# METHODS-Group/ProximalGalerkin

Hardware: AMD Instinct MI355X
Metric: proximal-Newton iterations/sec, 2048^2 P1 obstacle (LVPP Newton inner loop) (higher is better)
Workload: dtype f64; 1 GPU; 2048x2048 right-diagonal P1 obstacle problem on [-1,1]^2, phi_set obstacle, f=0, settings B: alpha double_exponential, alpha_max 100, tol 0.0001; snes_rtol 1e-6, Newton linear solves to true relative residual 1e-10; mixed_unknowns=8396802, step=one full LVPP solve from the zero state, parallelism=single

## Files before the change

proximalgalerkin_amd/csrc/pgx_api.hip:

```cpp
#include <algorithm>
#include <atomic>
#include <chrono>
#include <thread>
#include <cmath>
#include <cstdio>
#include <cstring>
#include <deque>
#include <map>
#include <mutex>
#include <string>
#include <vector>

#include "../../include/pgx.h"
#include "../../include/pgx_nd.h"
#include "pgx_comm.h"
#include "pgx_internal.h"

static thread_local std::string g_create_error;

struct DistLevel {
  int g, glo, H, ghi;
};
struct Dist {
  bool on = false;
  pgx_comm* comm = nullptr;
  int rank = 0, size = 1, ldist = 0, global_ny = 0;
  std::vector<DistLevel> L;
  GridLevel view{};
  int view_row0 = 0, view_glo = 0, view_H = 0, view_own0 = 0;
  long long n_halo = 0, n_allreduce = 0, n_vcycle = 0, n_krylov = 0;
  double* view_S = nullptr;
  size_t own_off = 0, own_cnt = 0;
  size_t eb = 0, eown_off = 0, eown_cnt = 0;
  size_t nk_field() const { return own_cnt + eown_cnt; }
  int cell0 = 0, ncell_own = 0;
  double *sb = nullptr, *wc = nullptr;
};

struct pgx_handle {
  int device = 0;
  Dist dist;
  hipStream_t st = nullptr;
  std::string err;
  int n = 0, nc = 0, nx = 0, ny = 0, nnz = 0;
  int degree = 1;
  int nd = 0;
  bool structured = false;
  QuadTab q{};
  double f = 0.0, alpha = 1.0;
  double* coords = nullptr;
  int32_t* cells = nullptr;
  uint8_t* mask = nullptr;
  double *gbc = nullptr, *bphi = nullptr;
  int32_t *rowptr = nullptr, *colm = nullptr, *v2c_ptr = nullptr, *v2c_ent = nullptr, *v2c_pos = nullptr;
  std::vector<int32_t> h_rowptr, h_col;
  size_t fill_lds = 0;
  double *Kv = nullptr, *Mv = nullptr, *Dv = nullptr;
  bool jac_valid = false;
  double* geoq = nullptr;
  float2* zf_out = nullptr;
  int z_f32 = 1;
  int f32_dbf16 = 1;
  bool dv_lean = false;
  int32_t *s_rowptr = nullptr, *s_colm = nullptr;
  double *s_K = nullptr, *s_M = nullptr, *s_D = nullptr;
  int s_nnz = 0;
  size_t s_fill_lds = 0;
  int32_t* s_blk = nullptr;
  int s_nblk = 0, spmv_bal = 1;
  uint8_t* s_code = nullptr;
  double* s_tab = nullptr;
  int s_ntab = 0, spmv_dict = 1;
  std::vector<int32_t> s_h_rowptr, s_h_col;
  QuadTab2 q2{};
  int32_t *cdofs = nullptr, *p2_v2c_ptr = nullptr, *p2_v2c_ent = nullptr, *p2_v2c_pos = nullptr;
  int32_t *v2e_ptr = nullptr, *v2e = nullptr, *edge_ends = nullptr;
  double *p2_xu = nullptr, *p2_xp = nullptr, *p2_ru = nullptr, *p2_rp = nullptr;
  double* p2_stash = nullptr;
  double *c1_bu = nullptr, *c1_bp = nullptr, *c1_xu = nullptr, *c1_xp = nullptr;
  int patch_nn = 0, p2_patch = 1, patch_nu = 2;
  int p2_fallback_its = 60, p2_fallbacks = 0;
  double patch_omega = 0.8;
  bool patch_fresh = false;
  std::vector<int32_t> patch_dof_host;
  int32_t *pdof = nullptr, *ppos = nullptr;
  void* pinv = nullptr;
  int patch_f32 = 1;
  struct P2St {
    int state = 0, enable = 1, dist_enable = 1, select = 1, i0 = 0, ni = 0, j0 = 0, nj = 0, nframe = 0, ref_rows[4] = {0, 0, 0, 0};
    P2StTab tab;
    double K[46];
    double* Dst = nullptr;
    float* Dstf = nullptr;
    int32_t* frame = nullptr;
    bool fresh = false;
  } p2st;
  float* s_Df = nullptr;
  int p2_resid_f32 = 1;
  int patch_sym = 1;
  double *p2_su = nullptr, *p2_sp = nullptr;
  double *x = nullptr, *xk = nullptr, *F = nullptr, *dx = nullptr, *xw = nullptr, *rhs = nullptr;
  int restart = 0;
  double *V = nullptr, *Z = nullptr, *w = nullptr, *d_small = nullptr, *partials = nullptr, *partials2 = nullptr;
  double* h_small = nullptr;
  double* h_small_dev = nullptr;
  unsigned long long* h_seq = nullptr;
  unsigned long long* h_seq_dev = nullptr;
  unsigned long long seq = 0;
  int lean_d = 1;
  int spmv_d4 = 1;
  int lazy_norm = 1;
  double rhs_scale = 1.0;
  const float* rhs_f32 = nullptr;
  int v_f32 = 1;
  double v_f32_gain = 1e-4;
  double v_f32_max = 1e30;
  int v_f32_min = 1000000;
  bool v_f32_off = false;
  int host_poll = 1;
  int gs_wide = 16;
  int fused_publish = 1;
  int fused_resid = 1;
  int lean_rhs = 1;
  int fused_step = 1;
  std::vector<GridLevel> lev;
  double *tmp_u = nullptr, *tmp_p = nullptr, *res_u = nullptr, *res_p = nullptr;
  double omega_now = 0.0;
  int coarse_sweeps = 4;
  int tail_start = -1;
  int xcd_remap = 2;
  int tail_verts = 1100;
  int spmv_stream = 1;
  int nu_coarse = 0;
  int fused_k3 = 1;
  int fused_legs = 1;
  int fused_min = 4000;
  int cgs_selective = 1;
  long cgs_skipped = 0, cgs_total = 0;
  double cgs_eta2 = 1e-4;
  TailArgs tail{};
  pgx_nd* lu = nullptr;
  pgx_comm* lu_comm = nullptr;
  double* Jmix = nullptr;
  bool dh_interior = false;
  int stag_its = 12;
  double stag_gain = 1e-4;
  int smooth_d32 = 0;
  int k6_max = 0;
  int mg_f32 = 1;
  int f32_min = 4000;
  int f32_k6_max = 300000;
  int f32_rr_max = 300000;
  int resid_grid = 1;
  int spmv_stencil = 1;
  bool lu_active = false;
  bool check_replicas = false;
  double *obs_partials = nullptr, *d_out6 = nullptr;
  int obs_blocks = 0;
  bool prof = false;
  double ms[8] = {0, 0, 0, 0, 0, 0, 0, 0};
  hipEvent_t e0 = nullptr, e1 = nullptr;
  std::vector<void*> allocs;
};

#define HIPCHK(call)                                                                            \
  do {                                                                                          \
    hipError_t e_ = (call);                                                                     \
    if (e_ != hipSuccess) {                                                                     \
      h->err = std::string(#call) + ": " + hipGetErrorString(e_);                               \
      return PGX_EHIP;                                                                          \
    }                                                                                           \
  } while (0)

template <typename T>
static int dalloc(pgx_handle* h, T** p, size_t count) {
  void* q = nullptr;
  hipError_t e = hipMalloc(&q, std::max<size_t>(count, 1) * sizeof(T));
  if (e != hipSuccess) {
    h->err = std::string("hipMalloc: ") + hipGetErrorString(e);
    return PGX_ENOMEM;
  }
  h->allocs.push_back(q);
  *p = (T*)q;
  return PGX_OK;
}
#define DALLOC(p, count)                         \
  do {                                           \
    int rc_ = dalloc(h, &(p), (size_t)(count));  \
    if (rc_) return rc_;                         \
  } while (0)

struct PhaseTimer {
  pgx_handle* h;
  int slot;
  PhaseTimer(pgx_handle* h_, int s) : h(h_), slot(s) {
    static const char* const names[8] = {"pgx:residual", "pgx:jacobian", "pgx:mg_setup/lu_factor", "pgx:spmv", "pgx:precond",
                                         "pgx:orthogonalise", "pgx:observables", "pgx:newton_solve"};
    pgx_roctx(names[s & 7]);
    if (h->prof) hipEventRecord(h->e0, h->st);
  }
  ~PhaseTimer() {
    pgx_roctx(nullptr);
    if (h->prof) {
      hipEventRecord(h->e1, h->st);
      hipEventSynchronize(h->e1);
      float ms = 0;
      hipEventElapsedTime(&ms, h->e0, h->e1);
      h->ms[slot] += ms;
    }
  }
};

namespace {
std::mutex g_tune_mu;
std::atomic<int> g_tune_gen{0};
std::map<std::string, const std::string*>& tune_table() {
  static std::map<std::string, const std::string*> t;
  return t;
}
std::deque<std::string>& tune_pool() {
  static std::deque<std::string> p;
  return p;
}
}
const char* pgx_tune(const char* name) {
  std::lock_guard<std::mutex> lk(g_tune_mu);
  auto& t = tune_table();
  auto it = t.find(name);
  return it == t.end() ? nullptr : it->second->c_str();
}
int pgx_tune_gen() { return g_tune_gen.load(std::memory_order_acquire); }
extern "C" int pgx_tuning_set(const char* key, const char* value) {
  if (!key || strncmp(key, "PGX_", 4) != 0) return PGX_EINVAL;
  std::lock_guard<std::mutex> lk(g_tune_mu);
  if (value) {
    const std::string* interned = nullptr;
    for (const std::string& s : tune_pool())
      if (s == value) interned = &s;
    if (!interned) {
      tune_pool().emplace_back(value);
      interned = &tune_pool().back();
    }
    tune_table()[key] = interned;
  } else {
    tune_table().erase(key);
  }
  g_tune_gen.fetch_add(1, std::memory_order_release);
  return PGX_OK;
}

extern "C" void pgx_default_opts(pgx_snes_opts* o) {
  o->snes_rtol = 1e-8;
  o->snes_atol = 1e-50;
  o->snes_stol = 1e-8;
  o->snes_divtol = 1e4;
  o->snes_max_it = 50;
  o->ksp_rtol = 0.0;
  o->ksp_max_it = 200;
  o->ksp_restart = 30;
  o->mg_nu = 6;
  o->mg_omega = 0.75;
  o->monitor = 0;
  o->pc_type = 0;
  o->linesearch = 0;
}

extern "C" const char* pgx_last_error(const pgx_handle* h) { return h ? h->err.c_str() : g_create_error.c_str(); }

static int build_plan(pgx_handle* h, const pgx_mesh* m, const std::vector<uint8_t>& hmask) {
  const int n = m->n_vertices, nc = m->n_cells;
  std::vector<int32_t> vptr(n + 1, 0);
  for (int c = 0; c < nc; ++c)
    for (int a = 0; a < 3; ++a) {
      const int v = m->cells[3 * c + a];
      if (v < 0 || v >= n) {
        h->err = "cell vertex id out of range";
        return PGX_EINVAL;
      }
      vptr[v + 1]++;
    }
  for (int i = 0; i < n; ++i) vptr[i + 1] += vptr[i];
  std::vector<int32_t> vent(vptr[n]), fillp(vptr.begin(), vptr.end() - 1);
  for (int c = 0; c < nc; ++c)
    for (int a = 0; a < 3; ++a) vent[fillp[m->cells[3 * c + a]]++] = c * 4 + a;
  std::vector<int32_t>& rowptr = h->h_rowptr;
  std::vector<int32_t>& col = h->h_col;
  rowptr.assign(n + 1, 0);
  col.clear();
  col.reserve((size_t)n * 7);
  std::vector<int32_t> tmp;
  for (int i = 0; i < n; ++i) {
    tmp.clear();
    for (int k = vptr[i]; k < vptr[i + 1]; ++k) {
      const int c = vent[k] >> 2;
      tmp.push_back(m->cells[3 * c]);
      tmp.push_back(m->cells[3 * c + 1]);
      tmp.push_back(m->cells[3 * c + 2]);
    }
    if (tmp.empty()) tmp.push_back(i);
    std::sort(tmp.begin(), tmp.end());
    tmp.erase(std::unique(tmp.begin(), tmp.end()), tmp.end());
    if (tmp.size() > 255) {
      h->err = "vertex degree > 255 unsupported";
      return PGX_EINVAL;
// ... 1401 lines not shown
    PhaseTimer t(h, 1);
    if (h->degree == 2) {
      pgxk_fill_rows_p2(h->st, 2, h->nd, h->s_fill_lds, h->s_rowptr, h->p2_v2c_ptr, h->p2_v2c_ent, h->p2_v2c_pos,
                        h->cdofs, h->coords, x + h->nd, h->q2, h->s_D, h->geoq);
      pgxk_fill_rows_p1_Dp2(h->st, h->n, h->fill_lds, h->rowptr, h->v2c_ptr, h->v2c_ent, h->v2c_pos, h->cdofs, h->coords,
                            x + h->nd, h->q2, h->Dv, h->geoq);
    } else if (h->resid_grid && h->structured && !h->lev.empty() && h->lev[0].uniform) {
      pgxk_resid_fill_grid(h->st, 1, h->lev[0], h->fill_lds, h->rowptr, h->v2c_ptr, h->v2c_ent, h->v2c_pos, h->cells, h->coords,
                           h->mask, h->gbc, h->bphi, x, h->xk, h->alpha, h->f, h->q, h->w, h->Dv, 1);
      h->dh_interior = true;
      h->dv_lean = false;
      have_d = true;
    } else {
      pgxk_fill_rows(h->st, 2, h->n, h->fill_lds, h->rowptr, h->v2c_ptr, h->v2c_ent, h->v2c_pos, h->cells, h->coords,
                     x + h->n, h->q, h->Dv, h->geoq);
    }
  }
  if (h->structured) {
    PhaseTimer t(h, 2);
    pgxk_csr_to_stencil_h(h->st, h->n, h->nx + 1, h->rowptr, h->colm, h->Dv, h->lev[0].Dh,
                          (have_d && h->degree == 1 && h->dh_interior) ? h->lev[0].ny : 0);
    h->dh_interior = false;
    if (h->lev[0].Dh32) pgxk_to_float(h->st, (size_t)4 * h->n, h->lev[0].Dh, h->lev[0].Dh32);
    if (h->lev[0].f32) pgxk_f_pack_d(h->st, h->lev[0]);
    if (h->lev[0].Dd4) pgxk_pack_d4(h->st, h->lev[0]);
    const int ld = h->dist.on ? h->dist.ldist : 0;
    for (size_t l = 1; l < h->lev.size(); ++l) {
      if (h->dist.on && (int)l == ld) {
        const Dist& D = h->dist;
        const GridLevel& G = h->lev[l];
#ifdef PGX_DSTEN_FLOAT
        h->err = "PGX_DSTEN_FLOAT builds do not support sharded handles";
        return PGX_EINVAL;
#else
        pgxk_rap7h(h->st, h->lev[l - 1], h->lev[l - 1].Dh, D.view, D.view_S);
        pgxk_view_to_global(h->st, 4, D.view.n, G.n, G.nx + 1, D.view_row0, D.view_own0, D.view_H, D.view_S, G.Dh);
        const int rc = allreduce_dev(h, G.Dh, (size_t)4 * G.n);
        if (rc) return rc;
#endif
      } else {
        pgxk_rap7h(h->st, h->lev[l - 1], h->lev[l - 1].Dh, h->lev[l], h->lev[l].Dh);
      }
      if (h->lev[l].f32) pgxk_f_pack_d(h->st, h->lev[l]);
    }
  }
  h->jac_valid = true;
  h->patch_fresh = false;
  h->p2st.fresh = false;
  return PGX_OK;
}

static bool p2st_ready(pgx_handle* h) {
  pgx_handle::P2St& S = h->p2st;
  if (S.state == 0 || !S.select || (h->dist.on && !S.dist_enable) || !h->s_K || !h->s_D) return false;
  static const int nt[4] = {19, 9, 9, 9}, off[4] = {0, 19, 28, 37};
  const size_t G = (size_t)h->n;
  if (S.state == 1) {
    S.state = 0;
    const std::vector<int32_t>& rp = h->s_h_rowptr;
    double kmax = 0.0, mmax = 0.0;
    for (int t = 0; t < 4; ++t) {
      const int p = rp[S.ref_rows[t]];
      if (hipMemcpy(S.K + off[t], h->s_K + p, sizeof(double) * nt[t], hipMemcpyDeviceToHost) != hipSuccess ||
          hipMemcpy(S.tab.M + off[t], h->s_M + p, sizeof(double) * nt[t], hipMemcpyDeviceToHost) != hipSuccess)
        return false;
    }
    for (int e = 0; e < 46; ++e) kmax = std::max(kmax, std::fabs(S.K[e])), mmax = std::max(mmax, std::fabs(S.tab.M[e]));
    S.tab.kmax = kmax, S.tab.mmax = mmax;
    for (int e = 0; e < 46; ++e) S.tab.aK[e] = S.K[e];
    int* d_fail = nullptr;
    if (hipMalloc((void**)&d_fail, sizeof(int)) != hipSuccess) return false;
    hipMemsetAsync(d_fail, 0, sizeof(int), h->st);
    pgxk_p2st_check(h->st, S.tab, h->nx, h->n, S.i0, S.ni, S.j0, S.nj, 1.0, 1e-12, h->s_rowptr, h->s_K, h->s_M, d_fail);
    int fail = 1;
    const hipError_t e1 = hipMemcpyAsync(&fail, d_fail, sizeof(int), hipMemcpyDeviceToHost, h->st);
    const hipError_t e2 = hipStreamSynchronize(h->st);
    hipFree(d_fail);
    if (e1 != hipSuccess || e2 != hipSuccess || fail) return false;
    void* q = nullptr;
    if (hipMalloc(&q, sizeof(double) * 46 * G) != hipSuccess) {
      (void)hipGetLastError();
      return false;
    }
    h->allocs.push_back(q);
    S.Dst = (double*)q;
    if (h->p2_resid_f32) {
      if (hipMalloc(&q, sizeof(float) * 46 * G) == hipSuccess) {
        h->allocs.push_back(q);
        S.Dstf = (float*)q;
      } else {
        (void)hipGetLastError();
      }
    }
    S.state = 2;
  }
  if (!S.fresh) {
    pgxk_p2st_pack(h->st, h->nx, h->n, S.i0, S.ni, S.j0, S.nj, G, h->s_rowptr, h->s_D, S.Dst, 0);
    if (S.Dstf) pgxk_p2st_pack(h->st, h->nx, h->n, S.i0, S.ni, S.j0, S.nj, G, h->s_rowptr, h->s_D, S.Dstf, 1);
    S.fresh = true;
  }
  for (int e = 0; e < 46; ++e) S.tab.aK[e] = h->alpha * S.K[e];
  return true;
}
static void p2st_apply(pgx_handle* h, const double* xu, const double* xp, const double* bu, const double* bp, double* yu, double* yp,
                       bool inner) {
  pgx_handle::P2St& S = h->p2st;
  const bool f32 = inner && S.Dstf;
  pgxk_p2st_apply(h->st, S.tab, h->nx, h->n, S.i0, S.ni, S.j0, S.nj, (size_t)h->n, f32 ? (const void*)S.Dstf : (const void*)S.Dst, f32, xu,
                  xp, bu, bp, yu, yp);
  pgxk_p2_rows_csr(h->st, S.nframe, S.frame, h->s_rowptr, h->s_colm, h->s_K, h->s_M, h->s_D, h->alpha, h->mask, xu, xp, bu, bp, yu, yp);
}

static void level_apply(pgx_handle* h, int l, int mode, const double* xu, const double* xp, const double* bu,
                        const double* bp, double omega, int first, double* yu, double* yp);
static void spmv_dev(pgx_handle* h, const double* x, double* y) {
  if (h->degree == 2 && h->spmv_stream && h->spmv_bal && p2st_ready(h)) {
    static PgxTuneInt bench_inner("PGX_P2ST_BENCH_INNER", 0);
    p2st_apply(h, x, x + h->nd, nullptr, nullptr, y, y + h->nd, bench_inner.get() != 0);
    return;
  }
  if (h->spmv_stencil && h->structured && h->degree == 1) {
    if (h->spmv_stencil == 2)
      level_apply(h, 0, 0, x, x + h->nd, nullptr, nullptr, 0.0, 0, y, y + h->nd);
    else
      pgxk_st_spmv(h->st, h->lev[0], h->alpha, x, x + h->nd, h->xcd_remap ? 1 : 0, y, y + h->nd);
    return;
  }
  if (h->spmv_stream && h->spmv_bal && h->s_blk)
    pgxk_bspmv_bal(h->st, h->nd, h->s_nblk, h->s_blk, h->s_rowptr, h->s_colm, h->s_K, h->s_M, h->s_code, h->s_tab, h->s_D, h->alpha, h->mask, x,
                   x + h->nd, nullptr, nullptr, h->xcd_remap ? 1 : 0, y, y + h->nd);
  else if (h->spmv_stream && 2 * h->s_fill_lds <= 100 * 1024)
    pgxk_bspmv_stream(h->st, h->nd, h->s_fill_lds, h->s_rowptr, h->s_colm, h->s_K, h->s_M, h->s_D, h->alpha, h->mask, x,
                      x + h->nd, h->xcd_remap ? 1 : 0, y, y + h->nd);
  else
    pgxk_bspmv(h->st, 0, h->nd, h->s_rowptr, h->s_colm, h->s_K, h->s_M, h->s_D, h->alpha, x, x + h->nd, nullptr,
               nullptr, 0.0, h->xcd_remap, y, y + h->nd);
}

static void level_apply(pgx_handle* h, int l, int mode, const double* xu, const double* xp, const double* bu,
                        const double* bp, double omega, int first, double* yu, double* yp) {
  if (l == 0 && !h->structured)
    pgxk_bspmv(h->st, mode, h->n, h->rowptr, h->colm, h->Kv, h->Mv, h->Dv, h->alpha, xu, xp, bu, bp, omega,
               first | h->xcd_remap, yu, yp);
  else
    pgxk_st_apply(h->st, mode, h->lev[l], h->alpha, xu, xp, bu, bp, omega, first | h->xcd_remap, yu, yp);
}

static void vcycle(pgx_handle* h, int l, const double* bu, const double* bp, double* outu, double* outp, int nu, double omega);

static const float2* vcycle_f(pgx_handle* h, int l, const double* bu, const double* bp, double* outu, double* outp, int nu,
                              double omega) {
  GridLevel& L = h->lev[l];
  GridLevel& C = h->lev[l + 1];
  const int K = (nu == 6 && L.n <= h->f32_k6_max && L.n <= h->f32_rr_max) ? 6 : ((nu % 3 == 0 && h->fused_k3) ? 3 : 2);
  const int nl = nu / K;
  const int remap = h->xcd_remap ? 1 : 0;
  float2 *cu = L.xf, *ou = L.xf2;
  const bool fuse = L.n <= h->f32_rr_max;
  float2* const cbf = C.f32 ? C.bf : nullptr;
  double* const cb64u = C.f32 ? nullptr : C.bu;
  double* const cb64p = C.f32 ? nullptr : C.bp;
  {
    const bool rr = fuse && nl == 1;
    const double bscale = (l == 0 && bu) ? h->rhs_scale : 1.0;
    const float* const b32 = (l == 0 && bu) ? h->rhs_f32 : nullptr;
    pgxk_f_smooth(h->st, K, 1, L, h->alpha, nullptr, bu, bp, rr ? &C : nullptr, nullptr, nullptr, nullptr, omega, remap, cu, nullptr,
                  nullptr, rr ? cbf : nullptr, rr ? cb64u : nullptr, rr ? cb64p : nullptr, bscale, b32, b32 ? b32 + L.n : nullptr);
  }
  for (int s = 1; s < nl; ++s) {
    const bool rr = fuse && s + 1 == nl;
    pgxk_f_smooth(h->st, K, 0, L, h->alpha, cu, nullptr, nullptr, rr ? &C : nullptr, nullptr, nullptr, nullptr, omega, remap, ou, nullptr,
                  nullptr, rr ? cbf : nullptr, rr ? cb64u : nullptr, rr ? cb64p : nullptr);
    std::swap(cu, ou);
  }
  if (!fuse) pgxk_f_resid_restrict(h->st, L, h->alpha, cu, C, remap, cbf, cb64u, cb64p);
  const float2* cf = nullptr;
  const double *cdu = nullptr, *cdp = nullptr;
  if (C.f32) {
    cf = vcycle_f(h, l + 1, nullptr, nullptr, nullptr, nullptr, nu, omega);
  } else {
    vcycle(h, l + 1, C.bu, C.bp, C.xu, C.xp, nu, omega);
    cdu = C.xu;
    cdp = C.xp;
  }
  for (int s = 0; s < nl; ++s) {
    const bool lastl = s + 1 == nl;
    float2* const zf = (lastl && l == 0) ? h->zf_out : nullptr;
    const bool out64 = lastl && outu && !zf;
    pgxk_f_smooth(h->st, K, 0, L, h->alpha, cu, nullptr, nullptr, s == 0 ? &C : nullptr, s == 0 ? cf : nullptr, s == 0 ? cdu : nullptr,
                  s == 0 ? cdp : nullptr, omega, remap, zf ? zf : ou, out64 ? outu : nullptr, out64 ? outp : nullptr);
    if (zf) return zf;
    std::swap(cu, ou);
  }
  return cu;
}
static inline bool f32_cycle_ok(const pgx_handle* h, int l, int nu) {
  return h->lev[l].f32 && h->fused_legs && l + 1 < (int)h->lev.size() && nu >= 2 && (nu % 2 == 0 || (nu % 3 == 0 && h->fused_k3));
}

static void vcycle(pgx_handle* h, int l, const double* bu, const double* bp, double* outu, double* outp, int nu,
                   double omega) {
  GridLevel& L = h->lev[l];
  if (f32_cycle_ok(h, l, nu)) {
    vcycle_f(h, l, bu, bp, outu, outp, nu, omega);
    return;
  }
  if (l > 0 && l == h->tail_start) {
    h->tail.nu = (h->nu_coarse > 0) ? std::min(nu, h->nu_coarse) : nu;
    h->tail.omega = omega;
    h->tail.alpha = h->alpha;
    h->tail.coarse_sweeps = h->coarse_sweeps;
    pgxk_mg_tail(h->st, h->tail);
    return;
  }
  const bool last = (l + 1 == (int)h->lev.size());
  double* Au = outu;
  double* Ap = outp;
  double* Bu = (l == 0) ? h->tmp_u : L.xu2;
  double* Bp = (l == 0) ? h->tmp_p : L.xp2;
  double* ru = (l == 0) ? h->res_u : L.ru;
  double* rp = (l == 0) ? h->res_p : L.rp;
  const int Kf = (nu % 3 == 0 && h->fused_k3) ? 3 : (nu % 2 == 0 ? 2 : 0);
  if (h->structured && !last && Kf && h->fused_legs && L.n >= h->fused_min) {
    GridLevel& C = h->lev[l + 1];
    const int remap = h->xcd_remap ? 1 : 0;
    const int Kl = (Kf == 3 && nu % 6 == 0 && L.n <= h->k6_max && pgxk_st_smooth6_ok(L)) ? 6 : Kf;
    const int nl = nu / Kl;
    double *cu = Bu, *cp = Bp, *ou = Au, *op = Ap;
    pgxk_st_smoothK(h->st, Kl, 0, L, h->alpha, nullptr, nullptr, nullptr, nullptr, nullptr, bu, bp, omega, remap, cu, cp);
    for (int s = 1; s < nl; ++s) {
      pgxk_st_smoothK(h->st, Kl, 1, L, h->alpha, cu, cp, nullptr, nullptr, nullptr, bu, bp, omega, remap, ou, op);
      std::swap(cu, ou);
      std::swap(cp, op);
    }
    pgxk_st_resid_restrict(h->st, L, h->alpha, cu, cp, bu, bp, C, remap, C.bu, C.bp);
    vcycle(h, l + 1, C.bu, C.bp, C.xu, C.xp, nu, omega);
    pgxk_st_smoothK(h->st, Kl, 1, L, h->alpha, cu, cp, &C, C.xu, C.xp, bu, bp, omega, remap, ou, op);
    std::swap(cu, ou);
    std::swap(cp, op);
    for (int s = 1; s < nl; ++s) {
      pgxk_st_smoothK(h->st, Kl, 1, L, h->alpha, cu, cp, nullptr, nullptr, nullptr, bu, bp, omega, remap, ou, op);
      std::swap(cu, ou);
      std::swap(cp, op);
    }
    if (cu != Au) {
      hipMemcpyAsync(Au, cu, sizeof(double) * L.n, hipMemcpyDeviceToDevice, h->st);
      hipMemcpyAsync(Ap, cp, sizeof(double) * L.n, hipMemcpyDeviceToDevice, h->st);
    }
    return;
  }
  if (l > 0 && h->nu_coarse > 0) nu = std::min(nu, h->nu_coarse);
  const int total = last ? (h->lev.size() == 1 ? 2 * nu : h->coarse_sweeps) : 2 * nu;
  bool toA = (total % 2) == 1;
  const double *cu = nullptr, *cp = nullptr;
  auto sweep = [&](int first) {
    double* tu = toA ? Au : Bu;
    double* tp = toA ? Ap : Bp;
    level_apply(h, l, 2, cu, cp, bu, bp, omega, first, tu, tp);
    cu = tu;
    cp = tp;
    toA = !toA;
  };
  if (last) {
    for (int s = 0; s < total; ++s) sweep(s == 0);
    return;
  }
  for (int s = 0; s < nu; ++s) sweep(s == 0);
  level_apply(h, l, 1, cu, cp, bu, bp, 0.0, 0, ru, rp);
  GridLevel& C = h->lev[l + 1];
  pgxk_restrict(h->st, L, ru, rp, C, C.bu, C.bp);
  vcycle(h, l + 1, C.bu, C.bp, C.xu, C.xp, nu, omega);
  pgxk_prolong_add(h->st, C, C.xu, C.xp, L, (double*)cu, (double*)cp);
  for (int s = 0; s < nu; ++s) sweep(0);
}

static int vcycle_dist_f(pgx_handle* h, int l, double* bu, double* bp, double* outu, double* outp, int need_out, int nu, double omega,
                         const float2** res);
static int vcycle_dist(pgx_handle* h, int l, double* bu, double* bp, double* outu, double* outp, int need_out, int nu,
                       double omega) {
  Dist& D = h->dist;
  GridLevel& L = h->lev[l];
  if (L.f32 && h->fused_legs) return vcycle_dist_f(h, l, bu, bp, outu, outp, need_out, nu, omega, nullptr);
  const int g = D.L[l].g;
  const int K = (nu % 3 == 0 && g >= 3 && h->fused_k3) ? 3 : 2;
  if (nu % K) {
    h->err = "sharded V-cycle: mg_nu must be even (or a multiple of 3 with deep enough ghost rows)";
    return PGX_EINVAL;
  }
  const int remap = h->xcd_remap ? 1 : 0;
  const int nl = nu / K;
  int rc = halo_level(h, l, bu, bp);
  if (rc) return rc;
  double *cu = (l == 0) ? h->tmp_u : L.xu2, *cp = (l == 0) ? h->tmp_p : L.xp2, *ou = outu, *op = outp;
  int xv;
  pgxk_st_smoothK(h->st, K, 0, L, h->alpha, nullptr, nullptr, nullptr, nullptr, nullptr, bu, bp, omega, remap, cu, cp);
  xv = g - K;
  auto more = [&](const GridLevel* C, const double* ccu, const double* ccp) -> int {
    if (xv < K) {
      const int r = halo_level(h, l, cu, cp);
      if (r) return r;
      xv = g;
    }
    pgxk_st_smoothK(h->st, K, 1, L, h->alpha, cu, cp, C, ccu, ccp, bu, bp, omega, remap, ou, op);
    std::swap(cu, ou);
    std::swap(cp, op);
    xv -= K;
    return PGX_OK;
// ... 1213 lines not shown
```

proximalgalerkin_amd/csrc/pgx_mg32.hip:

```cpp
#include <algorithm>

#include "pgx_internal.h"
#include "pgx_stencil.h"

#define F32_BLOCK 512
#ifndef F32_LEAN
#define F32_LEAN 0
#endif
#ifndef F32_WAVES_EU
#define F32_WAVES_EU 2
#endif
#define F32_RR_CYB 2
#define F32_TB 2

__device__ __forceinline__ float lane_shr1f(float x) {
  int v = __float_as_int(x);
  v = __builtin_amdgcn_update_dpp(v, v, 0x138, 0xf, 0xf, false);
  return __int_as_float(v);
}

typedef float f_v2f __attribute__((ext_vector_type(2)));
typedef __bf16 f_v2bf __attribute__((ext_vector_type(2)));
__device__ __forceinline__ uint32_t f_pack_bf16x2(float lo, float hi) {
  const f_v2f f = {lo, hi};
  return __builtin_bit_cast(uint32_t, __builtin_convertvector(f, f_v2bf));
}
__device__ __forceinline__ void f_pack_d(float4 q, float4& out) { out = q; }
__device__ __forceinline__ void f_pack_d(float4 q, uint2& out) { out = make_uint2(f_pack_bf16x2(q.x, q.y), f_pack_bf16x2(q.z, q.w)); }
__device__ __forceinline__ float4 f_unpack_d(float4 q) { return q; }
__device__ __forceinline__ float4 f_unpack_d(uint2 w) {
  return make_float4(__uint_as_float(w.x << 16), __uint_as_float(w.x & 0xffff0000u), __uint_as_float(w.y << 16),
                     __uint_as_float(w.y & 0xffff0000u));
}
__device__ __forceinline__ void f_zero_d(float4& q) { q = make_float4(0.f, 0.f, 0.f, 0.f); }
__device__ __forceinline__ void f_zero_d(uint2& w) { w = make_uint2(0u, 0u); }

template <class DT>
__global__ void __launch_bounds__(256) k_f_pack_d(int n, const dsten_t* __restrict__ Dh, DT* __restrict__ Dq) {
  const int v = blockIdx.x * blockDim.x + threadIdx.x;
  if (v >= n) return;
  const float big = 1e30f;
  f_pack_d(make_float4(fminf((float)Dh[v], big), fminf((float)Dh[(size_t)n + v], big), fminf((float)Dh[2 * (size_t)n + v], big),
                       fminf((float)Dh[3 * (size_t)n + v], big)),
           Dq[v]);
}
void pgxk_f_pack_d(hipStream_t st, const GridLevel& L) {
  if (L.dbf16)
    hipLaunchKernelGGL(k_f_pack_d<uint2>, dim3((L.n + 255) / 256), dim3(256), 0, st, L.n, L.Dh, (uint2*)L.Dq);
  else
    hipLaunchKernelGGL(k_f_pack_d<float4>, dim3((L.n + 255) / 256), dim3(256), 0, st, L.n, L.Dh, (float4*)L.Dq);
}

struct FCoef {
  float kv[7], mv[7], dv[7];
  int rowbc;
};
struct FConst {
  float kc[7], mc[7];
  float k0, k1, k3, k5, m0, m1, m3, m5;
  int uniform;
};
static inline FConst make_fconst(const GridLevel& L, double alpha) {
  FConst c;
  for (int s = 0; s < 7; ++s) {
    c.kc[s] = (float)alpha * (float)L.Kc[s];
    c.mc[s] = (float)L.Mc[s];
  }
  const float a = (float)alpha;
  c.k0 = a * (float)L.Kc[0];
  c.k1 = a * (float)(0.5 * (L.Kc[1] + L.Kc[2]));
  c.k3 = a * (float)(0.5 * (L.Kc[3] + L.Kc[4]));
  c.k5 = a * (float)(0.5 * (L.Kc[5] + L.Kc[6]));
  c.m0 = (float)L.Mc[0];
  c.m1 = (float)(0.5 * (L.Mc[1] + L.Mc[2]));
  c.m3 = (float)(0.5 * (L.Mc[3] + L.Mc[4]));
  c.m5 = (float)(0.5 * (L.Mc[5] + L.Mc[6]));
  c.uniform = L.uniform;
  return c;
}
template <class DT>
__device__ __forceinline__ void f_load_coef(int v, int i, int j, int nx, int ny, int n, const double* __restrict__ K,
                                            const double* __restrict__ M, const DT* __restrict__ Dq, const FConst& sc,
                                            const uint8_t* __restrict__ mask, float alpha, FCoef& c) {
  const int sx = nx + 1;
  if (sc.uniform && i > 0 && i < nx && j > 0 && j < ny) {
#pragma unroll
    for (int s = 0; s < 7; ++s) {
      c.kv[s] = sc.kc[s];
      c.mv[s] = sc.mc[s];
    }
  } else {
#pragma unroll
    for (int s = 0; s < 7; ++s) {
      c.kv[s] = alpha * (float)K[(size_t)s * n + v];
      c.mv[s] = (float)M[(size_t)s * n + v];
    }
  }
  const float4 q = f_unpack_d(Dq[v]);
  c.dv[0] = q.x;
  c.dv[1] = q.y;
  c.dv[3] = q.z;
  c.dv[5] = q.w;
  c.dv[2] = (i > 0) ? f_unpack_d(Dq[v - 1]).y : 0.f;
  c.dv[4] = (j > 0) ? f_unpack_d(Dq[v - sx]).z : 0.f;
  c.dv[6] = (i > 0 && j > 0) ? f_unpack_d(Dq[v - sx - 1]).w : 0.f;
  c.rowbc = mask[v];
}

__device__ __forceinline__ void f_jacobi(const FCoef& c, float omega, float au, float ap, float xur, float xpr, float buv, float bpv,
                                         float& yu, float& yp) {
  if (c.rowbc) au = xur;
  const float su = buv - au, sp = bpv - ap;
  float a = c.kv[0], b = c.mv[0];
  const float dd = c.dv[0];
  float om_u = omega;
  if (c.rowbc) {
    a = 1.f;
    b = 0.f;
    om_u = 1.f;
  }
  const float det = -a * dd - b * b;
  float du = 0.f, dpsi = 0.f;
  if (det != 0.f) {
    const float r = __builtin_amdgcn_rcpf(det);
    du = (-dd * su - b * sp) * r;
    dpsi = (-b * su + a * sp) * r;
  } else if (c.rowbc) {
    du = su;
  }
  yu = xur + om_u * du;
  yp = xpr + omega * dpsi;
}

template <int CADD>
__device__ __forceinline__ float2 f_add_coarse(float2 x, int gi, int gj, int nxc, const float2* __restrict__ cf,
                                               const double* __restrict__ cdu, const double* __restrict__ cdp) {
  if (CADD == 0) return x;
  const int sxc = nxc + 1;
  const int jc = gj >> 1, ic = gi >> 1;
  const unsigned c0 = (unsigned)(jc * sxc + ic), c1 = (unsigned)((jc + (gj & 1)) * sxc + ic + (gi & 1));
  if (CADD == 1) {
    const float2 a = cf[c0], b = cf[c1];
    x.x += 0.5f * (a.x + b.x);
    x.y += 0.5f * (a.y + b.y);
  } else {
    x.x += 0.5f * (float)(cdu[c0] + cdu[c1]);
    x.y += 0.5f * (float)(cdp[c0] + cdp[c1]);
  }
  return x;
}

struct FSmoothArgs {
  int nx, ny, n, nbnd, nxc, nyc, remap;
  RowmapGrid g;
  const double *K, *M;
  const void* Dq;
  int dbf16;
  const uint8_t *mask, *mask_c;
  const float2 *xf, *cf, *bf;
  const double *cdu, *cdp, *b64u, *b64p;
  float2 *bfo, *yf, *cbf;
  double *y64u, *y64p, *cb64u, *cb64p;
  float alpha, omega;
  double bscale;
  FConst sc;
  const float *b32u, *b32p;
// ... 181 lines not shown
  const int lane = threadIdx.x & 63;
  const int wave = __builtin_amdgcn_readfirstlane(threadIdx.x >> 6);
  const int gi = i0 + lane;
  const bool own_lane = lane >= HALO && lane < W - HALO;
  const DT* const Dq = static_cast<const DT*>(A.Dq);
  DT dw[R];
  float4 dq[R];
  float2 rb[R], xa[R];
  float kv[R][7], mv[R][7];
  bool in[R], bc[R];
#pragma unroll
  for (int k = 0; k < R; ++k) {
    const int lj = wave + NW * k, gj = j0 + lj;
    in[k] = lj < H0 && gi >= 0 && gi <= nx && gj >= 0 && gj <= ny;
    bc[k] = false;
    f_zero_d(dw[k]);
    rb[k] = xa[k] = make_float2(0.f, 0.f);
#pragma unroll
    for (int t = 0; t < 7; ++t) {
      kv[k][t] = A.sc.kc[t];
      mv[k][t] = A.sc.mc[t];
    }
    if (in[k]) {
      const int v = gj * sx + gi;
      dw[k] = Dq[v];
      bc[k] = A.mask[v] != 0;
      if (lj >= 1 && lj < H0 - 1) rb[k] = f_load_rhs<IO>(A, (unsigned)v);
      if (!FIRST) xa[k] = f_add_coarse<CADD>(A.xf[v], gi, gj, A.nxc, A.cf, A.cdu, A.cdp);
      if (!(A.sc.uniform && gi > 0 && gi < nx && gj > 0 && gj < ny)) {
#pragma unroll
        for (int t = 0; t < 7; ++t) {
          kv[k][t] = A.alpha * (float)A.K[(size_t)t * A.n + v];
          mv[k][t] = (float)A.M[(size_t)t * A.n + v];
        }
      }
    }
  }
#pragma unroll
  for (int k = 0; k < R; ++k) {
    const int lj = wave + NW * k;
    dq[k] = f_unpack_d(dw[k]);
    if (lj < H0) {
      if (!FIRST) img0[lj * W + lane] = make_float2(bc[k] ? 0.f : xa[k].x, xa[k].y);
      exch[lj * W + lane] = make_float2(dq[k].z, dq[k].w);
    }
  }
  __syncthreads();
  float d2[R], d4[R], d6[R], g0[R], g1[R], g2[R], g3[R];
#pragma unroll
  for (int k = 0; k < R; ++k) {
    const int lj = wave + NW * k;
    d2[k] = d4[k] = d6[k] = g0[k] = g1[k] = g2[k] = g3[k] = 0.f;
    if (lj >= 1 && lj < H0 - 1) {
      d2[k] = lane_shr1f(dq[k].y);
      d4[k] = exch[(lj - 1) * W + lane].x;
      d6[k] = exch[(lj - 1) * W + lane - 1].y;
      float a = kv[k][0], bm = mv[k][0], om_u = A.omega;
      if (bc[k]) {
        a = 1.f;
        bm = 0.f;
        om_u = 1.f;
      }
      const float det = -a * dq[k].x - bm * bm;
      if (det != 0.f) {
        const float r = __builtin_amdgcn_rcpf(det);
        g0[k] = om_u * (-dq[k].x * r);
        g1[k] = om_u * (-bm * r);
        g2[k] = A.omega * (-bm * r);
        g3[k] = A.omega * (a * r);
      } else if (bc[k]) {
        g0[k] = 1.f;
      }
    }
  }
#define F_ROWS_G(src, q, k, au, ap, x0)                                                                                            \
  const float2 x0 = src[q], x1_ = src[q + 1], x2_ = src[q - 1], x3_ = src[q + W], x4_ = src[q - W], x5_ = src[q + W + 1],          \
               x6_ = src[q - W - 1];                                                                                               \
  au = ((kv[k][0] * x0.x + kv[k][1] * x1_.x) + (kv[k][2] * x2_.x + kv[k][3] * x3_.x)) +                                            \
       ((kv[k][4] * x4_.x + kv[k][5] * x5_.x) + kv[k][6] * x6_.x) +                                                                \
       (((mv[k][0] * x0.y + mv[k][1] * x1_.y) + (mv[k][2] * x2_.y + mv[k][3] * x3_.y)) +                                           \
        ((mv[k][4] * x4_.y + mv[k][5] * x5_.y) + mv[k][6] * x6_.y));                                                               \
  ap = (((mv[k][0] * x0.x + mv[k][1] * x1_.x) + (mv[k][2] * x2_.x + mv[k][3] * x3_.x)) +                                           \
        ((mv[k][4] * x4_.x + mv[k][5] * x5_.x) + mv[k][6] * x6_.x)) -                                                              \
       (((dq[k].x * x0.y + dq[k].y * x1_.y) + (d2[k] * x2_.y + dq[k].z * x3_.y)) + ((d4[k] * x4_.y + dq[k].w * x5_.y) + d6[k] * x6_.y));
#pragma unroll
  for (int s = 1; s <= K; ++s) {
    const float2* const src = ((s - 1) & 1) ? img1 : img0;
    float2* const dst = (s & 1) ? img1 : img0;
    const bool act = lane >= s && lane < W - s;
#pragma unroll
    for (int k = 0; k < R; ++k) {
      const int lj = wave + NW * k;
      if (lj < s || lj >= H0 - s) continue;
      float au = 0.f, ap = 0.f, xur = 0.f, xpr = 0.f;
      if (!FIRST || s > 1) {
        F_ROWS_G(src, lj * W + lane, k, au, ap, x0)
        xur = x0.x;
        xpr = x0.y;
      }
      if (bc[k]) au = xur;
      const float su = rb[k].x - au, sp = rb[k].y - ap;
      const float ou = xur + fmaf(g0[k], su, g1[k] * sp);
      const float op = xpr + fmaf(g2[k], su, g3[k] * sp);
      if (act) {
        if (s == K && in[k] && lj >= HALO && lj < H0 - HALO && own_lane) {
          const int v = (j0 + lj) * sx + gi;
          if (IO == 1 || IO == 3) A.bfo[v] = rb[k];
          if (IO == 2) {
            A.y64u[v] = (double)ou;
            A.y64p[v] = (double)op;
          } else {
            A.yf[v] = make_float2(ou, op);
          }
        }
        if (s < K || RR) dst[lj * W + lane] = in[k] ? make_float2(bc[k] ? 0.f : ou, op) : make_float2(0.f, 0.f);
      }
    }
    if (s < K || RR) __syncthreads();
  }
  if (RR) {
    const float2* const xk = (K & 1) ? img1 : img0;
    float2* const rim = (K & 1) ? img0 : img1;
#pragma unroll
    for (int k = 0; k < R; ++k) {
      const int lj = wave + NW * k;
      if (lj < K + 1 || lj >= H0 - K - 1) continue;
      float au, ap;
      F_ROWS_G(xk, lj * W + lane, k, au, ap, x0)
      if (lane >= K + 1 && lane < W - K - 1)
        rim[lj * W + lane] = in[k] ? make_float2(bc[k] ? 0.f : rb[k].x - au, rb[k].y - ap) : make_float2(0.f, 0.f);
    }
    __syncthreads();
    const int sxc = A.nxc + 1, I0 = (tx * TX) >> 1, J0 = (ty * TY + sub * TB) >> 1;
    for (int cj = wave; cj < TB / 2; cj += NW)
      if (lane < TX / 2 && I0 + lane <= A.nxc && J0 + cj <= A.nyc) {
        const int q = (HALO + 2 * cj) * W + HALO + 2 * lane;
        const float2 r0 = rim[q], r1 = rim[q + 1], r2 = rim[q - 1], r3 = rim[q + W], r4 = rim[q - W], r5 = rim[q + W + 1],
                     r6 = rim[q - W - 1];
        float su = r0.x + 0.5f * (((r1.x + r2.x) + (r3.x + r4.x)) + (r5.x + r6.x));
        const float sp = r0.y + 0.5f * (((r1.y + r2.y) + (r3.y + r4.y)) + (r5.y + r6.y));
        const int C = (J0 + cj) * sxc + I0 + lane;
        if (A.mask_c[C]) su = 0.f;
        if (RR == 2) {
          A.cb64u[C] = (double)su;
          A.cb64p[C] = (double)sp;
        } else {
          A.cbf[C] = make_float2(su, sp);
        }
      }
  }
#undef F_ROWS_G
}

template <class DT, int TY, int K, bool FIRST, int IO, int CADD, int RR>
__global__ void __launch_bounds__(F32_BLOCK, RR ? 2 : F32_WAVES_EU) k_f_smooth(const FSmoothArgs A) {
  constexpr int W = 64, H0 = TY + 2 * (K + (RR ? 2 : 0)), PAD = W + 1;
  __shared__ float2 img_[3][H0 * W + 2 * PAD];
  const int blk = blockIdx.x;
  if (blk < A.nbnd)
    f_smooth_bnd<DT, TY, F32_TB, K, FIRST, IO, CADD, RR>(blk, A, img_[0] + PAD, img_[1] + PAD, img_[2] + PAD);
  else
    f_smooth_fast<DT, TY, K, FIRST, IO, CADD, RR>(xcd_block(blk - A.nbnd, gridDim.x - A.nbnd, A.remap), A, img_[0] + PAD, img_[1] + PAD, img_[2] + PAD);
}

template <class DT, int TY, int K>
static void launch_f_smooth_rr_t(hipStream_t st, int first, FSmoothArgs& A, int fast_ok) {
  const int rr = A.cbf ? 1 : 2;
  A.g = rowmap_grid<TY, K + 2>(A.nx, A.ny, fast_ok);
  const int nfast = A.g.nfx * A.g.nfy;
  A.nbnd = (A.g.ntx * A.g.nty - nfast) * (TY / F32_TB);
  const dim3 grid(A.nbnd + nfast), block(F32_BLOCK);
  if (first) {
    if (A.b32u) {
      if (rr == 1)
        hipLaunchKernelGGL((k_f_smooth<DT, TY, K, true, 3, 0, 1>), grid, block, 0, st, A);
      else
        hipLaunchKernelGGL((k_f_smooth<DT, TY, K, true, 3, 0, 2>), grid, block, 0, st, A);
    } else if (A.b64u) {
      if (rr == 1)
        hipLaunchKernelGGL((k_f_smooth<DT, TY, K, true, 1, 0, 1>), grid, block, 0, st, A);
      else
        hipLaunchKernelGGL((k_f_smooth<DT, TY, K, true, 1, 0, 2>), grid, block, 0, st, A);
    } else {
      if (rr == 1)
        hipLaunchKernelGGL((k_f_smooth<DT, TY, K, true, 0, 0, 1>), grid, block, 0, st, A);
      else
        hipLaunchKernelGGL((k_f_smooth<DT, TY, K, true, 0, 0, 2>), grid, block, 0, st, A);
    }
  } else {
    if (rr == 1)
      hipLaunchKernelGGL((k_f_smooth<DT, TY, K, false, 0, 0, 1>), grid, block, 0, st, A);
    else
      hipLaunchKernelGGL((k_f_smooth<DT, TY, K, false, 0, 0, 2>), grid, block, 0, st, A);
  }
}

template <int TY, int K>
static void launch_f_smooth_rr(hipStream_t st, int first, FSmoothArgs& A, int fast_ok) {
  if (A.dbf16)
    launch_f_smooth_rr_t<uint2, TY, K>(st, first, A, fast_ok);
  else
    launch_f_smooth_rr_t<float4, TY, K>(st, first, A, fast_ok);
}

template <class DT, int TY, int K>
static void launch_f_smooth_t(hipStream_t st, int first, FSmoothArgs& A, int fast_ok) {
  A.g = rowmap_grid<TY, K>(A.nx, A.ny, fast_ok);
  const int nfast = A.g.nfx * A.g.nfy;
  A.nbnd = (A.g.ntx * A.g.nty - nfast) * (TY / F32_TB);
  const dim3 grid(A.nbnd + nfast), block(F32_BLOCK);
  if (first) {
    if (A.b32u)
      hipLaunchKernelGGL((k_f_smooth<DT, TY, K, true, 3, 0, 0>), grid, block, 0, st, A);
    else if (A.b64u)
      hipLaunchKernelGGL((k_f_smooth<DT, TY, K, true, 1, 0, 0>), grid, block, 0, st, A);
    else
      hipLaunchKernelGGL((k_f_smooth<DT, TY, K, true, 0, 0, 0>), grid, block, 0, st, A);
    return;
  }
  const int cadd = A.cf ? 1 : (A.cdu ? 2 : 0);
  if (A.y64u) {
    if (cadd == 0)
      hipLaunchKernelGGL((k_f_smooth<DT, TY, K, false, 2, 0, 0>), grid, block, 0, st, A);
    else if (cadd == 1)
      hipLaunchKernelGGL((k_f_smooth<DT, TY, K, false, 2, 1, 0>), grid, block, 0, st, A);
    else
      hipLaunchKernelGGL((k_f_smooth<DT, TY, K, false, 2, 2, 0>), grid, block, 0, st, A);
  } else {
    if (cadd == 0)
      hipLaunchKernelGGL((k_f_smooth<DT, TY, K, false, 0, 0, 0>), grid, block, 0, st, A);
    else if (cadd == 1)
      hipLaunchKernelGGL((k_f_smooth<DT, TY, K, false, 0, 1, 0>), grid, block, 0, st, A);
    else
      hipLaunchKernelGGL((k_f_smooth<DT, TY, K, false, 0, 2, 0>), grid, block, 0, st, A);
  }
}

template <int TY, int K>
static void launch_f_smooth(hipStream_t st, int first, FSmoothArgs& A, int fast_ok) {
  if (A.dbf16)
    launch_f_smooth_t<uint2, TY, K>(st, first, A, fast_ok);
  else
    launch_f_smooth_t<float4, TY, K>(st, first, A, fast_ok);
}

static int f32_tile_rows(const GridLevel& L) {
  static PgxTuneInt t_ty("PGX_F32_TY", 0);
  const int ty = t_ty.get();
  if (ty == 4 || ty == 8 || ty == 16) return ty;
  return L.n >= 2000000 ? 16 : L.n >= 500000 ? 8 : 4;
}

void pgxk_f_smooth(hipStream_t st, int K, int first, const GridLevel& L, double alpha, const float2* xf, const double* b64u,
                   const double* b64p, const GridLevel* C, const float2* cf, const double* cdu, const double* cdp, double omega,
                   int remap, float2* yf, double* y64u, double* y64p, float2* cbf, double* cb64u, double* cb64p, double bscale,
                   const float* b32u, const float* b32p) {
  FSmoothArgs A;
  A.bscale = bscale;
  A.b32u = first ? b32u : nullptr;
  A.b32p = first ? b32p : nullptr;
  A.nyc = C ? C->ny : 0;
  A.mask_c = C ? C->mask : nullptr;
  A.cbf = cbf;
  A.cb64u = cb64u;
  A.cb64p = cb64p;
  A.nx = L.nx;
  A.ny = L.ny;
  A.n = L.n;
  A.nxc = C ? C->nx : 0;
  A.remap = remap;
  A.K = L.K;
  A.M = L.M;
  A.Dq = L.Dq;
  A.dbf16 = L.dbf16;
  A.mask = L.mask;
  A.xf = first ? nullptr : xf;
  A.cf = first ? nullptr : cf;
  A.cdu = first ? nullptr : cdu;
  A.cdp = first ? nullptr : cdp;
  A.b64u = first && !A.b32u ? b64u : nullptr;
  A.b64p = first && !A.b32u ? b64p : nullptr;
  A.bf = (A.b64u || A.b32u) ? nullptr : L.bf;
  A.bfo = (A.b64u || A.b32u) ? L.bf : nullptr;
  A.yf = yf;
  A.y64u = first ? nullptr : y64u;
  A.y64p = first ? nullptr : y64p;
  A.alpha = (float)alpha;
  A.omega = (float)omega;
  A.sc = make_fconst(L, alpha);
  const int ty = f32_tile_rows(L);
  if (K == 6) {
    if (cbf || cb64u)
      launch_f_smooth_rr<16, 6>(st, first, A, L.interior_free && (!C || C->interior_free));
    else
      launch_f_smooth<8, 6>(st, first, A, L.interior_free);
    return;
  }
  if (cbf || cb64u) {
    if (K == 3) {
      if (ty <= 8)
        launch_f_smooth_rr<8, 3>(st, first, A, L.interior_free && (!C || C->interior_free));
      else
        launch_f_smooth_rr<16, 3>(st, first, A, L.interior_free && (!C || C->interior_free));
    } else {
      if (ty <= 8)
        launch_f_smooth_rr<8, 2>(st, first, A, L.interior_free && (!C || C->interior_free));
      else
        launch_f_smooth_rr<16, 2>(st, first, A, L.interior_free && (!C || C->interior_free));
    }
    return;
  }
  if (K == 3) {
    if (ty == 4)
      launch_f_smooth<4, 3>(st, first, A, L.interior_free);
    else if (ty == 8)
      launch_f_smooth<8, 3>(st, first, A, L.interior_free);
    else
      launch_f_smooth<16, 3>(st, first, A, L.interior_free);
  } else {
    if (ty == 4)
      launch_f_smooth<4, 2>(st, first, A, L.interior_free);
    else if (ty == 8)
      launch_f_smooth<8, 2>(st, first, A, L.interior_free);
    else
      launch_f_smooth<16, 2>(st, first, A, L.interior_free);
  }
}

struct FRrArgs {
  int nx, ny, n, nbnd, nxc, nyc, remap;
  RrGrid g;
  const double *K, *M;
  const void* Dq;
  int dbf16;
  const uint8_t *mask, *mask_c;
  const float2 *xf, *bf;
  float2* cbf;
  double *cb64u, *cb64p;
  float alpha;
  FConst sc;
};

template <class DT, bool CB64>
__device__ __forceinline__ void f_rr_fast(int tx, int ty, const FRrArgs& A, float2* ximg, float2* rimg, float2* exch) {
  constexpr int W = 64, CX = 30, CY = 8, HX = 2 * CY + 3, HR = 2 * CY + 1, NW = F32_BLOCK / 64, R = (HX + NW - 1) / NW;
  const int sx = A.nx + 1, sxc = A.nxc + 1;
  const int I0 = tx * CX, J0 = ty * CY;
  const int i0 = 2 * I0 - 2, j0 = 2 * J0 - 2;
  const int lane = threadIdx.x & 63;
  const int wave = __builtin_amdgcn_readfirstlane(threadIdx.x >> 6);
  const int gi = i0 + lane;
  const bool act = lane >= 1 && lane < W - 1;
  const DT* const Dq = static_cast<const DT*>(A.Dq);
  float2 xa[R], rb[R];
  DT dw[R];
  float4 dq[R];
#pragma unroll
  for (int k = 0; k < R; ++k) {
    const int lj = wave + NW * k;
    if (lj < HX) {
      const unsigned v = (unsigned)((j0 + lj) * sx + gi);
      xa[k] = A.xf[v];
      if (lj <= HR) dw[k] = Dq[v];
      if (lj >= 1 && lj <= HR) rb[k] = A.bf[v];
    }
  }
#pragma unroll
  for (int k = 0; k < R; ++k) {
    const int lj = wave + NW * k;
    if (lj < HX) ximg[lj * W + lane] = xa[k];
    if (lj <= HR) {
      dq[k] = f_unpack_d(dw[k]);
      exch[lj * W + lane] = make_float2(dq[k].z, dq[k].w);
    }
  }
  __syncthreads();
  const float k0 = A.sc.k0, k1 = A.sc.k1, k3 = A.sc.k3, k5 = A.sc.k5, m0 = A.sc.m0, m1 = A.sc.m1, m3 = A.sc.m3, m5 = A.sc.m5;
#pragma unroll
  for (int k = 0; k < R; ++k) {
    const int lj = wave + NW * k;
    if (lj < 1 || lj > HR) continue;
    const float d2 = lane_shr1f(dq[k].y), d4 = exch[(lj - 1) * W + lane].x, d6 = exch[(lj - 1) * W + lane - 1].y;
    const int q = lj * W + lane;
    const float2 x0 = ximg[q], x1 = ximg[q + 1], x2 = ximg[q - 1], x3 = ximg[q + W], x4 = ximg[q - W], x5 = ximg[q + W + 1],
                 x6 = ximg[q - W - 1];
    const float u12 = x1.x + x2.x, u34 = x3.x + x4.x, u56 = x5.x + x6.x;
    const float p12 = x1.y + x2.y, p34 = x3.y + x4.y, p56 = x5.y + x6.y;
    const float au = (k0 * x0.x + k1 * u12) + (k3 * u34 + k5 * u56) + ((m0 * x0.y + m1 * p12) + (m3 * p34 + m5 * p56));
    const float ap = ((m0 * x0.x + m1 * u12) + (m3 * u34 + m5 * u56)) -
                     (((dq[k].x * x0.y + dq[k].y * x1.y) + (d2 * x2.y + dq[k].z * x3.y)) + ((d4 * x4.y + dq[k].w * x5.y) + d6 * x6.y));
    if (act) rimg[(lj - 1) * W + lane] = make_float2(rb[k].x - au, rb[k].y - ap);
  }
  __syncthreads();
  if (wave < CY && lane < CX) {
    const int q = (2 * wave + 1) * W + 2 * lane + 2;
    const float2 r0 = rimg[q], r1 = rimg[q + 1], r2 = rimg[q - 1], r3 = rimg[q + W], r4 = rimg[q - W], r5 = rimg[q + W + 1],
                 r6 = rimg[q - W - 1];
    const float su = r0.x + 0.5f * (((r1.x + r2.x) + (r3.x + r4.x)) + (r5.x + r6.x));
    const float sp = r0.y + 0.5f * (((r1.y + r2.y) + (r3.y + r4.y)) + (r5.y + r6.y));
    const int C = (J0 + wave) * sxc + I0 + lane;
    if (CB64) {
      A.cb64u[C] = (double)su;
      A.cb64p[C] = (double)sp;
    } else {
      A.cbf[C] = make_float2(su, sp);
    }
  }
}

template <class DT, bool CB64>
__device__ __forceinline__ void f_rr_bnd(int tx, int ty, int sub, const FRrArgs& A, float2* ximg, float2* rimg, float2* exch) {
  constexpr int W = 64, CX = 30, CY = 8, CYB = F32_RR_CYB, HX = 2 * CYB + 3, HR = 2 * CYB + 1, NW = F32_BLOCK / 64;
  static_assert(HX <= NW && CY % CYB == 0, "one image row per wave");
  const int nx = A.nx, ny = A.ny, sx = nx + 1, sxc = A.nxc + 1;
  const int I0 = tx * CX, J0 = ty * CY + sub * CYB;
  const int i0 = 2 * I0 - 2, j0 = 2 * J0 - 2;
  const int lane = threadIdx.x & 63;
  const int wave = __builtin_amdgcn_readfirstlane(threadIdx.x >> 6);
  const int gi = i0 + lane, lj = wave, gj = j0 + lj;
  const bool in = lj < HX && gi >= 0 && gi <= nx && gj >= 0 && gj <= ny;
  const bool act = lane >= 1 && lane < W - 1;
  DT dw;
  f_zero_d(dw);
  float2 rb = make_float2(0.f, 0.f), xa = make_float2(0.f, 0.f);
  float kv[7], mv[7];
  bool bc = false;
#pragma unroll
  for (int t = 0; t < 7; ++t) {
    kv[t] = A.sc.kc[t];
    mv[t] = A.sc.mc[t];
  }
  if (in) {
    const int v = gj * sx + gi;
    xa = A.xf[v];
    bc = A.mask[v] != 0;
    if (lj <= HR) dw = static_cast<const DT*>(A.Dq)[v];
    if (lj >= 1 && lj <= HR) {
      rb = A.bf[v];
      if (!(A.sc.uniform && gi > 0 && gi < nx && gj > 0 && gj < ny)) {
#pragma unroll
        for (int t = 0; t < 7; ++t) {
          kv[t] = A.alpha * (float)A.K[(size_t)t * A.n + v];
          mv[t] = (float)A.M[(size_t)t * A.n + v];
        }
      }
    }
  }
  const float4 dq = f_unpack_d(dw);
// ... 116 lines not shown
```

Before: 134.6 Newton iterations/s.

## Enable fused 6-sweep f32 smoother on large levels with taller tiles

Raises the level-size cap for the six-sweep fused f32 smoother so fine levels up to about 4.3M unknowns use it. Those levels therefore run it without the fused restriction, and the large-level tile height becomes 20 rows with a 4-row boundary band. The aim is fewer smoother kernel launches and less global traffic per sweep on the largest grids. The cost is a larger halo overhead per tile (6 rows each side), more shared memory, and possibly lower occupancy. It also adds an optional, default-off split launch for boundary and interior blocks.

```diff
diff --git a/proximalgalerkin_amd/csrc/pgx_api.hip b/proximalgalerkin_amd/csrc/pgx_api.hip
--- a/proximalgalerkin_amd/csrc/pgx_api.hip
+++ b/proximalgalerkin_amd/csrc/pgx_api.hip
@@ -149,7 +149,7 @@
   int k6_max = 0;
   int mg_f32 = 1;
   int f32_min = 4000;
-  int f32_k6_max = 300000;
+  int f32_k6_max = 4300000;
   int f32_rr_max = 300000;
   int resid_grid = 1;
   int spmv_stencil = 1;
@@ -1857,7 +1857,7 @@
                               double omega) {
   GridLevel& L = h->lev[l];
   GridLevel& C = h->lev[l + 1];
-  const int K = (nu == 6 && L.n <= h->f32_k6_max && L.n <= h->f32_rr_max) ? 6 : ((nu % 3 == 0 && h->fused_k3) ? 3 : 2);
+  const int K = (nu == 6 && L.n <= h->f32_k6_max) ? 6 : ((nu % 3 == 0 && h->fused_k3) ? 3 : 2);
   const int nl = nu / K;
   const int remap = h->xcd_remap ? 1 : 0;
   float2 *cu = L.xf, *ou = L.xf2;
diff --git a/proximalgalerkin_amd/csrc/pgx_mg32.hip b/proximalgalerkin_amd/csrc/pgx_mg32.hip
--- a/proximalgalerkin_amd/csrc/pgx_mg32.hip
+++ b/proximalgalerkin_amd/csrc/pgx_mg32.hip
@@ -10,8 +10,15 @@
 #ifndef F32_WAVES_EU
 #define F32_WAVES_EU 2
 #endif
+#ifndef F32_K6_SPLIT
+#define F32_K6_SPLIT 0
+#endif
+#ifndef F32_K6_TY_TOP
+#define F32_K6_TY_TOP 20
+#endif
 #define F32_RR_CYB 2
 #define F32_TB 2
+__host__ __device__ constexpr int f32_tb(int K, int RR) { return (K == 6 && !RR) ? 4 : F32_TB; }
 
 __device__ __forceinline__ float lane_shr1f(float x) {
   int v = __float_as_int(x);
@@ -499,13 +506,15 @@
 #undef F_ROWS_G
 }
 
-template <class DT, int TY, int K, bool FIRST, int IO, int CADD, int RR>
+template <class DT, int TY, int K, bool FIRST, int IO, int CADD, int RR, int PART = 0>
 __global__ void __launch_bounds__(F32_BLOCK, RR ? 2 : F32_WAVES_EU) k_f_smooth(const FSmoothArgs A) {
-  constexpr int W = 64, H0 = TY + 2 * (K + (RR ? 2 : 0)), PAD = W + 1;
+  constexpr int W = 64, H0 = (PART == 2 ? f32_tb(K, RR) : TY) + 2 * (K + (RR ? 2 : 0)), PAD = W + 1;
   __shared__ float2 img_[3][H0 * W + 2 * PAD];
   const int blk = blockIdx.x;
-  if (blk < A.nbnd)
-    f_smooth_bnd<DT, TY, F32_TB, K, FIRST, IO, CADD, RR>(blk, A, img_[0] + PAD, img_[1] + PAD, img_[2] + PAD);
+  if (PART == 2 || (PART == 0 && blk < A.nbnd))
+    f_smooth_bnd<DT, TY, f32_tb(K, RR), K, FIRST, IO, CADD, RR>(blk, A, img_[0] + PAD, img_[1] + PAD, img_[2] + PAD);
+  else if (PART == 1)
+    f_smooth_fast<DT, TY, K, FIRST, IO, CADD, RR>(xcd_block(blk, gridDim.x, A.remap), A, img_[0] + PAD, img_[1] + PAD, img_[2] + PAD);
   else
     f_smooth_fast<DT, TY, K, FIRST, IO, CADD, RR>(xcd_block(blk - A.nbnd, gridDim.x - A.nbnd, A.remap), A, img_[0] + PAD, img_[1] + PAD, img_[2] + PAD);
 }
@@ -550,36 +559,46 @@
     launch_f_smooth_rr_t<float4, TY, K>(st, first, A, fast_ok);
 }
 
+template <class DT, int TY, int K, bool FIRST, int IO, int CADD>
+static void launch_f_smooth_k(hipStream_t st, const FSmoothArgs& A, int nfast) {
+  const dim3 block(F32_BLOCK);
+  if constexpr (F32_K6_SPLIT && K == 6 && TY >= 12) {
+    if (A.nbnd) hipLaunchKernelGGL((k_f_smooth<DT, TY, K, FIRST, IO, CADD, 0, 2>), dim3(A.nbnd), block, 0, st, A);
+    if (nfast) hipLaunchKernelGGL((k_f_smooth<DT, TY, K, FIRST, IO, CADD, 0, 1>), dim3(nfast), block, 0, st, A);
+  } else {
+    hipLaunchKernelGGL((k_f_smooth<DT, TY, K, FIRST, IO, CADD, 0>), dim3(A.nbnd + nfast), block, 0, st, A);
+  }
+}
+
 template <class DT, int TY, int K>
 static void launch_f_smooth_t(hipStream_t st, int first, FSmoothArgs& A, int fast_ok) {
   A.g = rowmap_grid<TY, K>(A.nx, A.ny, fast_ok);
   const int nfast = A.g.nfx * A.g.nfy;
-  A.nbnd = (A.g.ntx * A.g.nty - nfast) * (TY / F32_TB);
-  const dim3 grid(A.nbnd + nfast), block(F32_BLOCK);
+  A.nbnd = (A.g.ntx * A.g.nty - nfast) * (TY / f32_tb(K, 0));
   if (first) {
     if (A.b32u)
-      hipLaunchKernelGGL((k_f_smooth<DT, TY, K, true, 3, 0, 0>), grid, block, 0, st, A);
+      launch_f_smooth_k<DT, TY, K, true, 3, 0>(st, A, nfast);
     else if (A.b64u)
-      hipLaunchKernelGGL((k_f_smooth<DT, TY, K, true, 1, 0, 0>), grid, block, 0, st, A);
+      launch_f_smooth_k<DT, TY, K, true, 1, 0>(st, A, nfast);
     else
-      hipLaunchKernelGGL((k_f_smooth<DT, TY, K, true, 0, 0, 0>), grid, block, 0, st, A);
+      launch_f_smooth_k<DT, TY, K, true, 0, 0>(st, A, nfast);
     return;
   }
   const int cadd = A.cf ? 1 : (A.cdu ? 2 : 0);
   if (A.y64u) {
     if (cadd == 0)
-      hipLaunchKernelGGL((k_f_smooth<DT, TY, K, false, 2, 0, 0>), grid, block, 0, st, A);
+      launch_f_smooth_k<DT, TY, K, false, 2, 0>(st, A, nfast);
     else if (cadd == 1)
-      hipLaunchKernelGGL((k_f_smooth<DT, TY, K, false, 2, 1, 0>), grid, block, 0, st, A);
+      launch_f_smooth_k<DT, TY, K, false, 2, 1>(st, A, nfast);
     else
-      hipLaunchKernelGGL((k_f_smooth<DT, TY, K, false, 2, 2, 0>), grid, block, 0, st, A);
+      launch_f_smooth_k<DT, TY, K, false, 2, 2>(st, A, nfast);
   } else {
     if (cadd == 0)
-      hipLaunchKernelGGL((k_f_smooth<DT, TY, K, false, 0, 0, 0>), grid, block, 0, st, A);
+      launch_f_smooth_k<DT, TY, K, false, 0, 0>(st, A, nfast);
     else if (cadd == 1)
-      hipLaunchKernelGGL((k_f_smooth<DT, TY, K, false, 0, 1, 0>), grid, block, 0, st, A);
+      launch_f_smooth_k<DT, TY, K, false, 0, 1>(st, A, nfast);
     else
-      hipLaunchKernelGGL((k_f_smooth<DT, TY, K, false, 0, 2, 0>), grid, block, 0, st, A);
+      launch_f_smooth_k<DT, TY, K, false, 0, 2>(st, A, nfast);
   }
 }
 
@@ -591,10 +610,17 @@
     launch_f_smooth_t<float4, TY, K>(st, first, A, fast_ok);
 }
 
-static int f32_tile_rows(const GridLevel& L) {
+static int f32_tile_rows(const GridLevel& L, int K) {
   static PgxTuneInt t_ty("PGX_F32_TY", 0);
   const int ty = t_ty.get();
+  if (K == 6) {
+    if (ty == 8 || ty == 12 || ty == 16 || ty == 20) return ty;
+    if (ty == 4) return 8;
+    return L.n <= 300000 ? 8 : F32_K6_TY_TOP;
+  }
   if (ty == 4 || ty == 8 || ty == 16) return ty;
+  if (ty == 12) return 8;
+  if (ty == 20) return 16;
   return L.n >= 2000000 ? 16 : L.n >= 500000 ? 8 : 4;
 }
 
@@ -635,12 +661,18 @@
   A.alpha = (float)alpha;
   A.omega = (float)omega;
   A.sc = make_fconst(L, alpha);
-  const int ty = f32_tile_rows(L);
+  const int ty = f32_tile_rows(L, K);
   if (K == 6) {
     if (cbf || cb64u)
       launch_f_smooth_rr<16, 6>(st, first, A, L.interior_free && (!C || C->interior_free));
+    else if (ty == 8)
+      launch_f_smooth<8, 6>(st, first, A, L.interior_free);
+    else if (ty == 12)
+      launch_f_smooth<12, 6>(st, first, A, L.interior_free);
+    else if (ty == 16)
+      launch_f_smooth<16, 6>(st, first, A, L.interior_free);
     else
-      launch_f_smooth<8, 6>(st, first, A, L.interior_free);
+      launch_f_smooth<20, 6>(st, first, A, L.interior_free);
     return;
   }
   if (cbf || cb64u) {
```

After: 145.8 Newton iterations/s (median of 6 runs). 8.3% higher.
